# meteorologytoday/XLab-FFTBarotropic

Measured on AMD Instinct MI355X. Metric: RK4 steps/sec, 4096x4096 periodic grid, higher is better.
Workload: dtype f32; 1 GPU; 4096x4096 kuo2004 initial field, nu=6.5, L=600 km, dt=0.75 s, 4 RK stages/step, fused HIP path; parallelism=single

## Files before the change

xlab-fftbarotropic_amd/csrc/fb_col_full.h:

```cpp
#pragma once
#include "fb_kernels.h"

#define CF_THREADS 1024
#define CF_X1_CF 16384
#define CF_X2_STR 68
#define CF_X2_CF (16 * 16 * CF_X2_STR)
#define CF_GX_CF 2048
#define CF_LDS_CF (CF_X2_CF + 512 + CF_GX_CF)
#define CF_LDS_BYTES (CF_LDS_CF * 8)

struct FullArgs {
    const cf *Tin;
    const cf *Zbase;
    cf *Zcur, *Acc, *Zout;
    cf *W4;
    long fstride;
    int P;
    int ntiles;
    int ntiles_run;
    int nsub;
    int stage;
    float nu, dt;
    SpecCoef coef;
    const cf *tw256;
    const cf *tw4096;
    long sub_rows;
    float wscale;
};

FB_DEV void cf_xchg_waves(cf *lds, cf *v, int w, int lane)
{
#pragma unroll
    for (int r = 0; r < 16; ++r) lds_wr(&lds[(r * 16 + w) * 64 + lane], v[r]);
    lds_barrier();
#pragma unroll
    for (int r = 0; r < 16; ++r) v[r] = lds_rd(&lds[(w * 16 + r) * 64 + lane]);
    lds_barrier();
}

template <bool SYNC>
FB_DEV void cf_xchg_lanes(cf *lds, cf *v, int w, int l, int c)
{
    cf *reg = lds + w * (16 * CF_X2_STR);
#pragma unroll
    for (int r = 0; r < 16; ++r) lds_wr(&reg[r * CF_X2_STR + l * 4 + c], v[r]);
    __builtin_amdgcn_wave_barrier();
#pragma unroll
    for (int r = 0; r < 16; ++r) v[r] = lds_rd(&reg[l * CF_X2_STR + r * 4 + c]);
    if (SYNC) lds_barrier();
    else { asm volatile("s_waitcnt lgkmcnt(0)" ::: "memory"); __builtin_amdgcn_wave_barrier(); }
}

#define CF_FENCE() __builtin_amdgcn_sched_barrier(0)
FB_DEV cf cf_mul(cf a, cf b) { return cmul_split(a, b); }
FB_DEV cf cf_mulc(cf a, cf b) { return cmulc_split(a, b); }

template <int DIR> FB_DEV void cf_bfly16(cf *v)
{
    fft4<DIR>(v[0], v[4], v[8], v[12]);  CF_FENCE();
    fft4<DIR>(v[1], v[5], v[9], v[13]);  CF_FENCE();
    fft4<DIR>(v[2], v[6], v[10], v[14]); CF_FENCE();
    fft4<DIR>(v[3], v[7], v[11], v[15]); CF_FENCE();
    v[5]  = mul_w16<1, DIR, true>(v[5]);  v[6]  = mul_w16<2, DIR, true>(v[6]);  v[7]  = mul_w16<3, DIR, true>(v[7]);
    v[9]  = mul_w16<2, DIR, true>(v[9]);  v[10] = mul_w16<4, DIR, true>(v[10]); v[11] = mul_w16<6, DIR, true>(v[11]);
    v[13] = mul_w16<3, DIR, true>(v[13]); v[14] = mul_w16<6, DIR, true>(v[14]); v[15] = mul_w16<9, DIR, true>(v[15]);
    CF_FENCE();
    fft4<DIR>(v[0], v[1], v[2], v[3]);     CF_FENCE();
    fft4<DIR>(v[4], v[5], v[6], v[7]);     CF_FENCE();
    fft4<DIR>(v[8], v[9], v[10], v[11]);   CF_FENCE();
    fft4<DIR>(v[12], v[13], v[14], v[15]); CF_FENCE();
    cf t;
    t = v[1];  v[1]  = v[4];  v[4]  = t;
    t = v[2];  v[2]  = v[8];  v[8]  = t;
    t = v[3];  v[3]  = v[12]; v[12] = t;
    t = v[6];  v[6]  = v[9];  v[9]  = t;
    t = v[7];  v[7]  = v[13]; v[13] = t;
    t = v[11]; v[11] = v[14]; v[14] = t;
}

template <int DIR>
FB_DEV void cf_fft4096(cf *lds, const cf *tabA, const cf *tabB, cf (*v)[16], int w, int l, int c, int lane)
{
    if (DIR < 0) {
#pragma unroll
        for (int col = 0; col < 2; ++col) {
            cf_bfly16<-1>(v[col]);
#pragma unroll
            for (int k1 = 1; k1 < 16; ++k1) { v[col][k1] = cf_mul(v[col][k1], tabB[w * k1]); if ((k1 & 3) == 3) CF_FENCE(); }
            cf_xchg_waves(lds, v[col], w, lane);
            CF_FENCE();
        }
        const cf a = tabA[l * w];
#pragma unroll
        for (int col = 0; col < 2; ++col) {
            cf_bfly16<-1>(v[col]);
            v[col][0] = cf_mul(v[col][0], a);
#pragma unroll
            for (int k2 = 1; k2 < 16; ++k2) { v[col][k2] = cf_mul(v[col][k2], cf_mul(a, tabB[l * k2])); if ((k2 & 3) == 3) CF_FENCE(); }
            cf_xchg_lanes<false>(lds, v[col], w, l, c);
            CF_FENCE();
        }
#pragma unroll
        for (int col = 0; col < 2; ++col) { cf_bfly16<-1>(v[col]); CF_FENCE(); }
    } else {
#pragma unroll
        for (int col = 0; col < 2; ++col) {
            cf_bfly16<+1>(v[col]);
#pragma unroll
            for (int lr = 1; lr < 16; ++lr) { v[col][lr] = cf_mulc(v[col][lr], cf_mul(tabA[lr * w], tabB[lr * l])); if ((lr & 3) == 3) CF_FENCE(); }
            if (col == 0) cf_xchg_lanes<false>(lds, v[col], w, l, c);
            else cf_xchg_lanes<true>(lds, v[col], w, l, c);
            CF_FENCE();
        }
#pragma unroll
        for (int col = 0; col < 2; ++col) {
            cf_bfly16<+1>(v[col]);
#pragma unroll
            for (int wr = 1; wr < 16; ++wr) { v[col][wr] = cf_mulc(v[col][wr], tabB[wr * w]); if ((wr & 3) == 3) CF_FENCE(); }
            cf_xchg_waves(lds, v[col], w, lane);
            CF_FENCE();
        }
#pragma unroll
        for (int col = 0; col < 2; ++col) { cf_bfly16<+1>(v[col]); CF_FENCE(); }
    }
}

FB_DEV float4 cf_ld4(const void *ubase, unsigned voff) { return *reinterpret_cast<const float4 *>(static_cast<const char *>(ubase) + voff); }
FB_DEV void cf_st4(void *ubase, unsigned voff, float4 x) { *reinterpret_cast<float4 *>(static_cast<char *>(ubase) + voff) = x; }
FB_DEV void cf_st4_w4(void *ubase, unsigned voff, float4 x) { st4<true>(static_cast<char *>(ubase) + voff, x); }

template <int STAGE, int NSUB>
__global__ void __launch_bounds__(CF_THREADS) k_col_full(FullArgs a)
{
    extern __shared__ __attribute__((aligned(16))) unsigned char smem_raw[];
    cf *lds = reinterpret_cast<cf *>(smem_raw);
    cf *tabB = lds + CF_X2_CF, *tabA = tabB + 256;
    float *gxt = reinterpret_cast<float *>(tabA + 256);
    const int tid = threadIdx.x, lane = tid & 63, l = lane >> 2, c = lane & 3;
    const int w = __builtin_amdgcn_readfirstlane(tid >> 6);

    constexpr int nsub = NSUB;
    const int ntg = gridDim.x / nsub;
    const int k1 = NSUB == 1 ? 0 : blockIdx.x / ntg, bt = blockIdx.x - k1 * ntg;
    int tile = bt;
    if ((ntg & 7) == 0) tile = (bt & 7) * (ntg >> 3) + (bt >> 3);
    if (tile >= a.ntiles_run) return;

    const int ky0 = tile * 8 + 2 * c;
    const unsigned voff_m = (unsigned)((l * a.P + 2 * c) * (int)sizeof(cf));
    const size_t ubase_m = ((size_t)(k1 * a.sub_rows + 16 * w) * a.P + (size_t)tile * 8) * sizeof(cf);
    const size_t rstep = (size_t)256 * a.P * sizeof(cf);
    const unsigned voff_s = (unsigned)(lane * (int)sizeof(float4));
    const size_t ubase_s = ((((size_t)k1 * (a.ntiles + 1) + tile) * 16) * CF_THREADS + (size_t)w * 64) * sizeof(float4);
    const size_t sstep = (size_t)CF_THREADS * sizeof(float4);

    constexpr bool PRIME = STAGE == 4;
    cf v[2][16];
    {
        const char *src = reinterpret_cast<const char *>(a.Tin) + ubase_m;
        float4 tin[16];
        if (!PRIME) {
#pragma unroll
            for (int i = 0; i < 16; ++i) tin[i] = ld4<true>(src + i * rstep + voff_m);
        }
        float g4[4];
#pragma unroll
        for (int i = 0; i < 4; ++i) g4[i] = a.coef.gx[nsub * (tid + i * CF_THREADS) + k1];
        if (tid < 256) { tabB[tid] = a.tw256[tid]; tabA[tid] = a.tw4096[tid]; }
#pragma unroll
        for (int i = 0; i < 4; ++i) {
            const int ik = tid + i * CF_THREADS;
            gxt[((ik >> 4) & 15) + 16 * (ik & 15) + (ik & ~255)] = g4[i];
        }
        if (!PRIME) {
#pragma unroll
            for (int i = 0; i < 16; ++i) { v[0][i] = cf_make(tin[i].x, tin[i].y); v[1][i] = cf_make(tin[i].z, tin[i].w); }
        }
    }
    __syncthreads();
    if (!PRIME) cf_fft4096<-1>(lds, tabA, tabB, v, w, l, c, lane);

    const char *Z0 = reinterpret_cast<const char *>(a.Zbase) + ubase_s;
    char *ZC = reinterpret_cast<char *>(a.Zcur) + ubase_s, *AC = reinterpret_cast<char *>(a.Acc) + ubase_s,
         *ZO = reinterpret_cast<char *>(a.Zout) + ubase_s;
    const float gya = a.coef.gy[ky0], gyb = a.coef.gy[ky0 + 1];
    auto ky2_of = [](float g) { asm volatile("" : "+v"(g)); return (double)g * (double)g; };
    constexpr bool PRIME_ = STAGE == 4;
    const bool pada = PRIME_ && ky0 >= a.coef.hy, padb = PRIME_ && ky0 + 1 >= a.coef.hy;
    constexpr int stage = STAGE;
    const float nu = a.nu, dt = a.dt, hdt = (stage == 2) ? a.dt : a.dt / 2.0f;
    constexpr int DEPTH = STAGE == 0 ? 2 : 1;
#ifndef CF_REMAKE_ZC
#define CF_REMAKE_ZC 1
#endif
    constexpr bool REMAKE_ZC = CF_REMAKE_ZC && STAGE == 1;
    float4 q0[DEPTH], q1[DEPTH], q2[DEPTH];
    auto load_k3 = [&](int k3) {
        const int sl = k3 % DEPTH;
        q0[sl] = ld4<false>(Z0 + k3 * sstep + voff_s);
        if (stage != 0) q2[sl] = ld4<true>(AC + k3 * sstep + voff_s);
        if (stage != 0 && !REMAKE_ZC) q1[sl] = ld4<false>(ZC + k3 * sstep + voff_s);
    };
    if (!PRIME) {
#pragma unroll
        for (int k3 = 0; k3 < DEPTH; ++k3) load_k3(k3);
    }
#pragma unroll
    for (int k3 = 0; k3 < (PRIME ? 0 : 16); ++k3) {
        const int sl = k3 % DEPTH;
        const int ik2 = w + 256 * k3 + 16 * l, ikx = nsub * ik2 + k1;
        const float gx = gxt[l + 16 * w + 256 * k3];
        const double kx2 = (double)gx * (double)gx;
        const float lapa = (float)(-(kx2 + ky2_of(gya))), lapb = (float)(-(kx2 + ky2_of(gyb)));
        const float mska = coef_mask(a.coef, ikx, ky0), mskb = coef_mask(a.coef, ikx, ky0 + 1);
        const float4 z0 = q0[sl];
        float4 zc = z0;
        if (REMAKE_ZC) {
            const float4 ac = q2[sl];
            zc = make_float4(__builtin_fmaf(ac.x, hdt, z0.x), __builtin_fmaf(ac.y, hdt, z0.y), __builtin_fmaf(ac.z, hdt, z0.z), __builtin_fmaf(ac.w, hdt, z0.w));
        } else if (stage != 0) zc = q1[sl];
        float4 k;
        k.x = (v[0][k3].x + (zc.x * lapa) * nu) * mska; k.y = (v[0][k3].y + (zc.y * lapa) * nu) * mska;
        k.z = (v[1][k3].x + (zc.z * lapb) * nu) * mskb; k.w = (v[1][k3].y + (zc.w * lapb) * nu) * mskb;
        float4 acc, zn;
        if (stage == 0) {
            acc = k;
            zn = make_float4(__builtin_fmaf(k.x, hdt, z0.x), __builtin_fmaf(k.y, hdt, z0.y), __builtin_fmaf(k.z, hdt, z0.z), __builtin_fmaf(k.w, hdt, z0.w));
        } else if (stage < 3) {
            const float4 ac = q2[sl];
            acc = make_float4(ac.x + 2.0f * k.x, ac.y + 2.0f * k.y, ac.z + 2.0f * k.z, ac.w + 2.0f * k.w);
            zn = make_float4(z0.x + k.x * hdt, z0.y + k.y * hdt, z0.z + k.z * hdt, z0.w + k.w * hdt);
        } else {
            const float4 ac = q2[sl];
            acc = ac;
            zn = make_float4(z0.x + (ac.x + k.x) * dt / 6.0f, z0.y + (ac.y + k.y) * dt / 6.0f,
                             z0.z + (ac.z + k.z) * dt / 6.0f, z0.w + (ac.w + k.w) * dt / 6.0f);
        }
        v[0][k3] = cf_make(zn.x, zn.y); v[1][k3] = cf_make(zn.z, zn.w);
        if (k3 + DEPTH < 16) load_k3(k3 + DEPTH);
        if (stage < 3) { st4<true>(AC + k3 * sstep + voff_s, acc); cf_st4(ZC + k3 * sstep, voff_s, zn); }
        else cf_st4(ZO + k3 * sstep, voff_s, zn);
        CF_FENCE();
    }

    const char *ZN = PRIME ? Z0 : (stage < 3 ? ZC : ZO);
#pragma unroll 1
    for (int f = 0; f < 4; ++f) {
        if (f > 0 || PRIME) {
            const unsigned vs = (unsigned)launder((int)voff_s);
#pragma unroll
            for (int k3 = 0; k3 < 16; ++k3) {
                const float4 z = cf_ld4(ZN + k3 * sstep, vs);
                v[0][k3] = cf_make(z.x, z.y); v[1][k3] = cf_make(z.z, z.w);
            }
        }
        const bool psi = f >= 2, use_gx = (f == 0 || f == 3);
        const int lkx = launder(l);
#pragma unroll
        for (int k3 = 0; k3 < 16; ++k3) {
            cf za = v[0][k3], zb = v[1][k3];
            const float gx = gxt[16 * w + 256 * k3 + lkx];
            if (psi) {
                const double kx2 = (double)gx * (double)gx;
                const float lia = (nsub * (w + 256 * k3 + 16 * l) + k1 == 0 && ky0 == 0) ? 1.0f : (float)(-(kx2 + ky2_of(gya)));
                const float lib = (float)(-(kx2 + ky2_of(gyb)));
                za = pada ? cf_make(0.f, 0.f) : cf_make(za.x / lia, za.y / lia);
                zb = padb ? cf_make(0.f, 0.f) : cf_make(zb.x / lib, zb.y / lib);
            }
            const float ka = (use_gx ? gx : gya) * a.wscale, kb = (use_gx ? gx : gyb) * a.wscale;
            v[0][k3] = cf_make(-za.y * ka, za.x * ka);
            v[1][k3] = cf_make(-zb.y * kb, zb.x * kb);
            CF_FENCE();
        }
        cf_fft4096<+1>(lds, tabA, tabB, v, w, l, c, lane);
        char *dst = reinterpret_cast<char *>(a.W4) + (size_t)f * a.fstride * sizeof(cf) + ubase_m;
        const unsigned vm = (unsigned)launder((int)voff_m);
#pragma unroll
        for (int i = 0; i < 16; ++i)
            cf_st4_w4(dst + i * rstep, vm, make_float4(v[0][i].x, v[0][i].y, v[1][i].x, v[1][i].y));
    }
}

template <bool TO_FULL>
__global__ void __launch_bounds__(256) k_full_relayout(const cf *__restrict__ in, cf *__restrict__ out, int P, int N1, int N2, int ntiles, int nsub, int hy)
{
    const size_t total = (size_t)nsub * (ntiles + 1) * 16 * CF_THREADS * 2;
    for (size_t idx = (size_t)blockIdx.x * blockDim.x + threadIdx.x; idx < total; idx += (size_t)gridDim.x * blockDim.x) {
        const int col = (int)(idx & 1);
        const int tid = (int)((idx >> 1) & (CF_THREADS - 1));
        const int k3 = (int)((idx >> 11) & 15);
        const int st = (int)(idx >> 15);
        const int k1 = st / (ntiles + 1), tile = st - k1 * (ntiles + 1);
        const int w = tid >> 6, l = (tid >> 2) & 15, c = tid & 3;
        const int kx = nsub * (w + 16 * l + 256 * k3) + k1, ky = tile * 8 + 2 * c + col;
        const int cc = kx % N1, d = kx / N1;
        const size_t p3 = (size_t)(N2 * cc + d) * P + ky;
        if (ky >= hy) { if (TO_FULL) out[idx] = cf_make(0.f, 0.f); continue; }
        if (TO_FULL) out[idx] = in[p3]; else out[p3] = in[idx];
    }
}
```

xlab-fftbarotropic_amd/csrc/fb_kernels.h:

```cpp
#pragma once
#include "fb_fft_core.h"

struct SpecCoef {
    const float  *gx;
    const double *kx2;
    const float  *gy;
    const double *ky2;
    double gws;
    int nx, hy;
    int gws_i;
};

FB_DEV float coef_lap(const SpecCoef &c, int i, int j) { return (float)(-(c.kx2[i] + c.ky2[j])); }
FB_DEV float coef_mask(const SpecCoef &c, int i, int j)
{
    const int ii = i < c.nx - i ? i : c.nx - i;
    const int r2 = ii * ii + j * j;
    return (r2 >= c.gws_i || j >= c.hy) ? 0.0f : 1.0f;
}

enum { OP_GRADX = 0, OP_GRADY = 1, OP_LAP = 2, OP_INVLAP = 3, OP_DEALIAS = 4 };

template <int OP>
__global__ void __launch_bounds__(256) k_spec_op(SpecCoef c, const cf *__restrict__ in, cf *__restrict__ out, int hy, size_t total)
{
#pragma clang fp contract(off)
    for (size_t idx = (size_t)blockIdx.x * blockDim.x + threadIdx.x; idx < total; idx += (size_t)gridDim.x * blockDim.x) {
        const int i = (int)(idx / hy), j = (int)(idx - (size_t)i * hy);
        cf a = in[idx], r;
        if (OP == OP_GRADX) { float k = c.gx[i]; r = cf_make(-a.y * k, a.x * k); }
        else if (OP == OP_GRADY) { float k = c.gy[j]; r = cf_make(-a.y * k, a.x * k); }
        else if (OP == OP_LAP) { float k = coef_lap(c, i, j); r = cf_make(a.x * k, a.y * k); }
        else if (OP == OP_INVLAP) { float k = (i == 0 && j == 0) ? 1.0f : coef_lap(c, i, j);
                                    r = cf_make(a.x / k, a.y / k); }
        else { float k = coef_mask(c, i, j); r = cf_make(a.x * k, a.y * k); }
        out[idx] = r;
    }
}

__global__ void __launch_bounds__(256) k_scale_real(float *d, float s, int divide, size_t n)
{
#pragma clang fp contract(off)
    for (size_t i = (size_t)blockIdx.x * blockDim.x + threadIdx.x; i < n; i += (size_t)gridDim.x * blockDim.x)
        d[i] = divide ? d[i] / s : d[i] * s;
}

__global__ void __launch_bounds__(256) k_jacobian(const float *__restrict__ u, const float *__restrict__ v,
                                                  const float *__restrict__ dx, const float *__restrict__ dy,
                                                  const float *__restrict__ src, float *__restrict__ out, size_t n)
{
#pragma clang fp contract(off)
    for (size_t i = (size_t)blockIdx.x * blockDim.x + threadIdx.x; i < n; i += (size_t)gridDim.x * blockDim.x) {
        float s = src ? src[i] : 0.0f;
        out[i] = -u[i] * dx[i] - v[i] * dy[i] + s;
    }
}

__global__ void __launch_bounds__(256) k_spec_axpy(const float *__restrict__ base, const float *__restrict__ x, float a,
                                                   float *__restrict__ out, size_t n)
{
#pragma clang fp contract(off)
    for (size_t i = (size_t)blockIdx.x * blockDim.x + threadIdx.x; i < n; i += (size_t)gridDim.x * blockDim.x)
        out[i] = base[i] + x[i] * a;
}

__global__ void __launch_bounds__(256) k_rk4_combine(const float *__restrict__ base, const float *__restrict__ k1,
                                                     const float *__restrict__ k2, const float *__restrict__ k3,
                                                     const float *__restrict__ k4, float dt, float *__restrict__ out, size_t n)
{
#pragma clang fp contract(off)
    for (size_t i = (size_t)blockIdx.x * blockDim.x + threadIdx.x; i < n; i += (size_t)gridDim.x * blockDim.x)
        out[i] = base[i] + (k1[i] + 2.0f * k2[i] + 2.0f * k3[i] + k4[i]) * dt / 6.0f;
}

template <bool TO_PRIVATE>
__global__ void __launch_bounds__(256) k_spec_relayout(const cf *__restrict__ in, cf *__restrict__ out, int nx, int hy, int P, int N1, int N2)
{
    const size_t total = (size_t)nx * P;
    for (size_t idx = (size_t)blockIdx.x * blockDim.x + threadIdx.x; idx < total; idx += (size_t)gridDim.x * blockDim.x) {
        const int row = (int)(idx / P), col = (int)(idx - (size_t)row * P);
        const int c = row / N2, d = row - c * N2, kx = c + N1 * d;
        if (TO_PRIVATE) out[idx] = col < hy ? in[(size_t)kx * hy + col] : cf_make(0.f, 0.f);
        else if (col < hy) out[(size_t)kx * hy + col] = in[idx];
    }
}

template <int MODE>
__global__ void __launch_bounds__(256) k_psi_private(SpecCoef c, cf *__restrict__ z, int P, int N1, int N2, int ky0)
{
#pragma clang fp contract(off)
    const size_t total = (size_t)c.nx * P;
    for (size_t idx = (size_t)blockIdx.x * blockDim.x + threadIdx.x; idx < total; idx += (size_t)gridDim.x * blockDim.x) {
        const int row = (int)(idx / P), col = (int)(idx - (size_t)row * P);
        const int cc = row / N2, d = row - cc * N2, i = cc + N1 * d, j = ky0 + col;
        cf a = z[idx];
        if (j >= c.hy) { z[idx] = cf_make(0.f, 0.f); continue; }
        const float li = (i == 0 && j == 0) ? 1.0f : coef_lap(c, i, j);
        a = cf_make(a.x / li, a.y / li);
        if (MODE == 1) { const float k = c.gy[j]; a = cf_make(-a.y * k, a.x * k); }
        if (MODE == 2) { const float k = c.gx[i]; a = cf_make(-a.y * k, a.x * k); }
        z[idx] = a;
    }
}

__global__ void __launch_bounds__(256) k_ow_spec(SpecCoef c, const cf *zin, cf *z, long fstride, int P, int N1, int N2, int ky0)
{
#pragma clang fp contract(off)
    const size_t total = (size_t)c.nx * P;
    for (size_t idx = (size_t)blockIdx.x * blockDim.x + threadIdx.x; idx < total; idx += (size_t)gridDim.x * blockDim.x) {
        const int row = (int)(idx / P), col = (int)(idx - (size_t)row * P);
        const int cc = row / N2, d = row - cc * N2, i = cc + N1 * d, j = ky0 + col;
        cf a = zin[idx], xx = cf_make(0.f, 0.f), yy = xx, xy = xx;
        if (j < c.hy) {
            const float li = (i == 0 && j == 0) ? 1.0f : coef_lap(c, i, j);
            a = cf_make(a.x / li, a.y / li);
            const float kx = c.gx[i], ky = c.gy[j];
            const cf ax = cf_make(-a.y * kx, a.x * kx), ay = cf_make(-a.y * ky, a.x * ky);
            xx = cf_make(-ax.y * kx, ax.x * kx);
            yy = cf_make(-ay.y * ky, ay.x * ky);
            xy = cf_make(-ay.y * kx, ay.x * kx);
        }
        z[idx] = xx; z[idx + fstride] = yy; z[idx + 2 * fstride] = xy;
    }
}

__global__ void __launch_bounds__(256) k_pres_spec(SpecCoef c, const cf *zin, cf *z, long fstride, int P, int N1, int N2, int ky0)
{
#pragma clang fp contract(off)
    const size_t total = (size_t)c.nx * P;
    for (size_t idx = (size_t)blockIdx.x * blockDim.x + threadIdx.x; idx < total; idx += (size_t)gridDim.x * blockDim.x) {
        const int row = (int)(idx / P), col = (int)(idx - (size_t)row * P);
        const int cc = row / N2, d = row - cc * N2, i = cc + N1 * d, j = ky0 + col;
        cf a = zin[idx], xx = cf_make(0.f, 0.f), yy = xx, xy = xx;
        if (j < c.hy) {
            const float li = (i == 0 && j == 0) ? 1.0f : coef_lap(c, i, j);
            a = cf_make(a.x / li, a.y / li);
            const float kx = c.gx[i], ky = c.gy[j], mk = coef_mask(c, i, j);
            const cf ax = cf_make(-a.y * kx, a.x * kx), ay = cf_make(-a.y * ky, a.x * ky);
            xx = cf_make(-ax.y * kx, ax.x * kx);
            yy = cf_make(-ay.y * ky, ay.x * ky);
            xy = cf_make(-ay.y * kx, ay.x * kx);
            xx = cf_make(xx.x * mk, xx.y * mk);
            yy = cf_make(yy.x * mk, yy.y * mk);
            xy = cf_make(xy.x * mk, xy.y * mk);
        }
        z[idx] = xx; z[idx + fstride] = yy; z[idx + 2 * fstride] = xy;
    }
}

__global__ void __launch_bounds__(256) k_pres_solve(SpecCoef c, const cf *__restrict__ zin, cf *__restrict__ l, float rho, float f, int P, int N1, int N2,
                                                    int ky0)
{
#pragma clang fp contract(off)
    const size_t total = (size_t)c.nx * P;
    for (size_t idx = (size_t)blockIdx.x * blockDim.x + threadIdx.x; idx < total; idx += (size_t)gridDim.x * blockDim.x) {
        const int row = (int)(idx / P), col = (int)(idx - (size_t)row * P);
        const int cc = row / N2, d = row - cc * N2, i = cc + N1 * d, j = ky0 + col;
        if (j >= c.hy) { l[idx] = cf_make(0.f, 0.f); continue; }
        const float lap = coef_lap(c, i, j), li = (i == 0 && j == 0) ? 1.0f : lap;
        const cf v = zin[idx], L = l[idx];
        const cf psi = cf_make(v.x / li, v.y / li);
        const cf t = cf_make(psi.x * lap, psi.y * lap);
        const float ax = t.x * f, ay = t.y * f, bx = L.x + L.x, by = L.y + L.y;
        const float qx = rho * (bx + ax), qy = rho * (by + ay);
        l[idx] = cf_make(qx / li, qy / li);
    }
}

__global__ void k_pres_ref(const float *__restrict__ p, long at, float *__restrict__ dst, int world)
{
    const int i = blockIdx.x * blockDim.x + threadIdx.x;
    if (i < world) dst[i] = at >= 0 ? p[at] : 0.0f;
}
template <bool V4>
__global__ void __launch_bounds__(256) k_pres_sub(float *__restrict__ p, size_t n, const float *__restrict__ ref)
{
    const float r = *ref;
    const size_t stride = (size_t)gridDim.x * blockDim.x;
    if (V4) {
        float4 *p4 = reinterpret_cast<float4 *>(p);
        for (size_t i = (size_t)blockIdx.x * blockDim.x + threadIdx.x; i < n / 4; i += stride) {
            float4 v = p4[i];
            v.x -= r; v.y -= r; v.z -= r; v.w -= r;
            p4[i] = v;
        }
    } else {
        for (size_t i = (size_t)blockIdx.x * blockDim.x + threadIdx.x; i < n; i += stride) p[i] -= r;
    }
}

template <bool TO_TM>
__global__ void __launch_bounds__(256) k_state_relayout(const cf *__restrict__ in, cf *__restrict__ out, int nx, int P, int N2)
{
    const int R1 = N2 >> 3, NLB = N2 >> 2, ntc = P >> 4;
    const size_t total = (size_t)nx * P;
    for (size_t idx = (size_t)blockIdx.x * blockDim.x + threadIdx.x; idx < total; idx += (size_t)gridDim.x * blockDim.x) {
        const int row = (int)(idx / P), col = (int)(idx - (size_t)row * P);
        const int cb = row / N2, d = row - cb * N2, ct = col >> 4, c = col & 15;
        const int q = d / R1, rem = d - q * R1, h = rem & 3, sidx = rem >> 2, e = 8 * sidx + q;
        const size_t tile = (size_t)cb * ntc + ct;
        const size_t tm = ((tile * (NLB / 2) + (e >> 1)) * 64 + (16 * h + c)) * 2 + (e & 1);
        if (TO_TM) out[tm] = in[idx]; else out[idx] = in[tm];
    }
}

enum { ROW_FUSED = 0, ROW_INV = 1, ROW_FWD = 2, ROW_OW = 3, ROW_KEFF = 4, ROW_PRES = 5 };

FB_DEV float pres_curv_point(float pxx, float pyy, float pxy)
{
#pragma clang fp contract(off)
    const float a = pxx * pyy, b = pxy * pxy;
    return a - b;
}

FB_DEV void ow_point(float pxx, float pyy, float pxy, float *w_out, float *tau_out, size_t i)
{
#pragma clang fp contract(off)
    const float w = 4.0f * (pxy * pxy - pxx * pyy);
    if (w_out) w_out[i] = w;
    if (tau_out) tau_out[i] = w > 0.0f ? 2.0f / sqrtf(w) : __builtin_inff();
}

FB_DEV void keff_grad2_point(float zx, float zy, float *g_out, size_t i)
{
#pragma clang fp contract(off)
    g_out[i] = zx * zx + zy * zy;
}

struct RowView {
    const cf *a, *b, *f;
    long fstrA, fstrB, fstrF;
    long sstrA, sstrB, sstrF;
    int ka, ka0, kb, kf;
    int katot;
    unsigned magA, magF;
};
struct RowArgs {
    RowView M;
    RowView T;
    int t_frozen;
    const float *src;
    const int *src_nz;
    const float *rin;
    float *rout;
    int x0, nx;
    float scale;
    int prescaled;
    const cf *tw_bwd, *tw_fwd;
    long sub_rows;
    const cf *tw_x;
};

FB_DEV float *row_rout2(const RowArgs &a) { return const_cast<float *>(a.rin); }

__global__ void __launch_bounds__(256) k_src_row_flags(const float *__restrict__ src, int *__restrict__ flags, int ny)
{
    const float4 *row = reinterpret_cast<const float4 *>(src + (size_t)blockIdx.x * ny);
    int any = 0;
    for (int i = threadIdx.x; i < ny / 4; i += 256) { const float4 v = row[i]; any |= (v.x != 0.f) | (v.y != 0.f) | (v.z != 0.f) | (v.w != 0.f); }
    any = __syncthreads_or(any);
    if (threadIdx.x == 0) flags[blockIdx.x] = any ? 1 : 0;
}

template <int N> struct RowCfg {
    static constexpr int T = N / 16;
    static constexpr int G = T >= 256 ? 1 : 256 / T;
    static constexpr int THREADS = T * G;
    static constexpr bool HALFX = false;
    static constexpr int LSTR = HALFX ? (N / 2 + N / 32) : (N + N / 16);
    static constexpr bool DMA = N >= 1024 && N <= 8192;
    static constexpr int GSTR = LSTR + (DMA ? N : 0);
    static constexpr bool RES = RowRes<N>::value;
    static constexpr bool SHARE = RES && RowPlanSymmetric<N>::value;
    static constexpr int TWL_B = RowTwSrc<N, false, RES>::LDS_CF, TWL_F = SHARE ? 0 : RowTwSrc<N, true, RES>::LDS_CF;
    static constexpr bool PAIR2 = N <= 1024 && G >= 2;
    static constexpr int VALB = PAIR2 ? G * 8 * T : 0;
    static constexpr size_t LDS_BYTES = ((size_t)G * GSTR + TWL_B + TWL_F + VALB) * sizeof(cf);
    static constexpr int MIN_WAVES = HALFX ? 3 : (THREADS == 256 ? 2 : (THREADS == 512 ? 2 : 4));
};

template <bool SLAB>
FB_DEV const cf *row_ptr(const RowView &v, int field, int row, int k)
{
    if (!SLAB) return v.a + (size_t)field * v.fstrA + (size_t)row * v.ka + k;
    if (k < v.katot) {
        const int s = (int)__umulhi((unsigned)k, v.magA), w = k - s * v.ka;
        if (v.kb == 0) return v.a + (size_t)field * v.fstrA + (size_t)s * v.sstrA + (size_t)row * v.ka + w;
        const bool inb = w >= v.ka0;
        const cf *base = inb ? v.b : v.a;
        const long fstr = inb ? v.fstrB : v.fstrA, sstr = inb ? v.sstrB : v.sstrA;
        const int kc = inb ? v.kb : v.ka0, wc = inb ? w - v.ka0 : w;
        return base + (size_t)field * fstr + (size_t)s * sstr + (size_t)row * kc + wc;
    }
    const int kk = k - v.katot, s = (int)__umulhi((unsigned)kk, v.magF);
    return v.f + (size_t)field * v.fstrF + (size_t)s * v.sstrF + (size_t)row * v.kf + (kk - s * v.kf);
}
template <bool SLAB> FB_DEV bool row_keep(const RowView &v, int t_frozen, int k) { return !SLAB || t_frozen || k < v.katot; }

template <int N, bool SLAB, int TAG = 0>
FB_DEV void row_load_pair(cf *reg, int t, const RowView &v, int fA, int fB, int rowA, int rowB)
{
    constexpr int T = N / 16, R0 = RowTw<N, false>::radix(0);
#pragma unroll
    for (int e = 0; e < 16; ++e) {
        const int i = ord_i<R0>(e);
        if (i < 8) {
            const int k = t + i * T;
            const cf a = *row_ptr<SLAB>(v, fA, rowA, k), b = *row_ptr<SLAB>(v, fB, rowB, k);
            reg[e] = (i == 0 && t == 0) ? cf_make(a.x, b.x) : cf_make(a.x - b.y, a.y + b.x);
        } else {
            const int k = (16 - i) * T - t;
            const cf a = *row_ptr<SLAB>(v, fA, rowA, k), b = *row_ptr<SLAB>(v, fB, rowB, k);
            reg[e] = (i == 8 && t == 0) ? cf_make(a.x, b.x) : cf_make(a.x + b.y, b.x - a.y);
        }
    }
}

template <int N, bool SLAB>
FB_DEV void row_store_pair(cf *lds, int t, const cf *reg, bool valid, const RowView &v, int t_frozen, int rowA, int rowB)
{
    constexpr int T = N / 16, RL = RowTw<N, true>::radix(RowPlan<N>::S - 1);
    constexpr int HOFF = RowCfg<N>::HALFX ? N / 2 : 0;
// ... 619 lines not shown
```

xlab-fftbarotropic_amd/csrc/fftbaro.hip:

```cpp
#include <hip/hip_runtime.h>
#include <algorithm>
#include <cmath>
#include <cstdio>
#include <cstdlib>
#include <cstring>
#include <mutex>
#include <set>
#include <string>
#include <type_traits>
#include <utility>
#include <vector>

#include "../../include/fftbaro.h"
#include "fb_kernels.h"
#include "fb_keff.h"
#include "fb_azim.h"
#include "fb_census.h"
#include "fb_spectra.h"
#include "fb_tracer.h"
#include "fb_particles.h"
#include "fb_tangent.h"
#include "fb_adjoint.h"
#include "fb_col_full.h"
#include "fb_row3.h"
// ... 767 lines not shown
        if (verbose) fprintf(stderr, "fftbaro: pitch probe P=%d %.4f ms\n", P0 + 16 * k, tbest[k]);
        if (tbest[k] < best * 0.99f) { best = tbest[k]; bestP = P0 + 16 * k; }
    }
    if (verbose) fprintf(stderr, "fftbaro: pitch %d -> %d\n", P0, bestP);
    c->P = c->KA = c->katot = c->grp[0].ncols = bestP;
    finish_groups(c);
    hipEventDestroy(e0); hipEventDestroy(e1);
    hipFree(buf);
    hipGetLastError();
    return FB_OK;
}

static int ensure_scratch(fb_ctx *c)
{
    if (!c->d_scratch) {
        hipError_t e = hipMalloc((void **)&c->d_scratch, priv_elems(c) * sizeof(cf));
        if (e != hipSuccess) return fail(FB_ENOMEM, "scratch allocation failed");
    }
    return FB_OK;
}

static unsigned magic_div(int d) { return d > 0 ? (unsigned)((1ull << 32) / (unsigned)d) + 1u : 0u; }
static RowView view_single(const fb_ctx *c, const cf *base, long fstride)
{
    RowView v; memset(&v, 0, sizeof(v));
    v.a = v.b = v.f = base; v.fstrA = v.fstrB = v.fstrF = fstride; v.ka = v.ka0 = c->P; v.kb = 0; v.kf = 16; v.katot = 0x7fffffff;
    return v;
}
static RowView view_slab(const fb_ctx *c, const cf *const *bufs, int nfields)
{
    RowView v; memset(&v, 0, sizeof(v));
    v.a = bufs[0]; v.b = c->nact > 1 ? bufs[1] : bufs[0]; v.f = c->KF > 0 ? bufs[c->nact] : bufs[0];
    v.ka = c->KA; v.ka0 = c->grp[0].ncols; v.kb = c->nact > 1 ? c->grp[1].ncols : 0; v.kf = c->KF > 0 ? c->KF : 16;
    v.katot = c->katot;
    v.fstrA = (long)c->XL * v.ka0; v.fstrB = (long)c->XL * v.kb; v.fstrF = (long)c->XL * v.kf;
    v.sstrA = (long)nfields * v.fstrA; v.sstrB = (long)nfields * v.fstrB; v.sstrF = (long)nfields * v.fstrF;
    v.magA = magic_div(v.ka); v.magF = magic_div(v.kf);
    return v;
}
static RowArgs row_args_base(const fb_ctx *c)
{
    RowArgs a; memset(&a, 0, sizeof(a));
    a.x0 = 0; a.nx = c->XL; a.tw_bwd = c->d_tw_row_bwd; a.tw_fwd = c->d_tw_row_fwd; a.t_frozen = 1;
    return a;
}

static int r2c_private(fb_ctx *c, const float *d_real, cf *dst)
{
    RowArgs a = row_args_base(c); a.rin = d_real; a.T = view_single(c, dst, 0);
    int rc;
    if ((rc = launch_row<ROW_FWD>(c, a))) return rc;
    if ((rc = launch_col_strided<-1>(c, c->grp[0], dst, 1, 0))) return rc;
    return launch_col_block<-1>(c, c->grp[0], dst, 1, 0);
}

static int c2r_private(fb_ctx *c, cf *work, float *d_real, float scale)
{
    int rc;
    if ((rc = launch_col_block<+1>(c, c->grp[0], work, 1, 0))) return rc;
    if ((rc = launch_col_strided<+1>(c, c->grp[0], work, 1, 0))) return rc;
    RowArgs a = row_args_base(c); a.M = view_single(c, work, 0); a.rout = d_real; a.scale = scale;
    return launch_row<ROW_INV>(c, a);
}

static bool state_tm(const fb_ctx *c) { return c->N2 >= 32; }
static int state_convert(fb_ctx *c, const ColGroup &G, const cf *in, cf *out, bool to_tm)
{
    if (G.ncols == 0) return FB_OK;
    if (!state_tm(c)) { HIPCHK(hipMemcpyAsync(out, in, grp_elems(c, G) * sizeof(cf), hipMemcpyDeviceToDevice, c->stream)); return FB_OK; }
    const size_t total = grp_elems(c, G);
    return launch_n(c, to_tm ? k_state_relayout<true> : k_state_relayout<false>, total, in, out, c->nx, G.ncols, c->N2);
}

static int relayout(fb_ctx *c, const cf *in, cf *out, bool to_private)
{
    const size_t total = priv_elems(c);
    return launch_n(c, to_private ? k_spec_relayout<true> : k_spec_relayout<false>, total, in, out, c->nx, c->hy, c->P, c->N1, c->N2);
}

extern "C" int fb_r2c(fb_ctx *c, const float *d_in, float *d_out)
{
    if (!c || !d_in || !d_out) return fail(FB_EINVAL, "fb_r2c: NULL");
    NEED_SINGLE(c);
    int rc;
    if ((rc = ensure_scratch(c))) return rc;
    HIPCHK(hipMemsetAsync(c->d_scratch, 0, priv_elems(c) * sizeof(cf), c->stream));
    if ((rc = r2c_private(c, d_in, c->d_scratch))) return rc;
    return relayout(c, c->d_scratch, (cf *)d_out, false);
}

extern "C" int fb_c2r(fb_ctx *c, const float *d_in, float *d_out, int normalize)
{
    if (!c || !d_in || !d_out) return fail(FB_EINVAL, "fb_c2r: NULL");
    NEED_SINGLE(c);
    int rc;
    if ((rc = ensure_scratch(c))) return rc;
    if ((rc = relayout(c, (const cf *)d_in, c->d_scratch, true))) return rc;
    const float scale = normalize ? 1.0f / (float)((size_t)c->nx * c->ny) : 1.0f;
    return c2r_private(c, c->d_scratch, d_out, scale);
}

struct GroupBufs { cf *ZA, *ZB, *ACC, *w4_send, *w4_recv, *t_send, *t_recv; };

struct Beside { cf *c0[3], *c1[3], *acc[3]; };

struct fb_model {
    fb_ctx *c;
    float nu, dt;
    GroupBufs gb[3];
    bool phase_flow;
    XPass xpass;
    bool prescale;
    bool use_graph, warmed;
    hipGraphExec_t graph_exec;
    const float *graph_src; hipStream_t graph_stream;
    float *src;
    int *src_nz;
    cf *rec_work[3], *rec_send[3];
    float *keff_fields;
    void *keff_red; size_t keff_red_cap;
    float *azim_fields;
    void *azim_red; size_t azim_red_cap;
    int *cs_label, *cs_ids;
    int2 *cs_part;
    float *pres_ref;
    unsigned char rec_work_nf[3], rec_send_nf[3];
    void *spec_red;
    int primed;
    Beside tr;
    float kappa;
    bool tracer;
    double *pt; int pt_n;
    float *pt_uv;
    double *pd;
    long long steps, pd_steps0;
    Beside tg[FB_TANGENTS_MAX];
    int tg_n;
    cf *tg_j[3];
    double *tg_red;
    cf *ad_tape; int ad_depth, ad_fill;
    Beside ad;
    float *ad_real;
    bool adjoint;
};

#include "fb_transport.h"
struct fb_slab {
    fb_ctx *c;
    fb_model *m;
    fb_transport tp;
    bool connected, owns_streams;
    hipStream_t comp, comm;
    hipEvent_t ev_f[4], ev_r[8], ev_w4, ev_t, ev_tg[2], ev_rows_done, ev_fwd_done, ev_misc[2];
    int nfg, nch;
    int ncg;
    int step_ops;
};
#include "fb_entry.h"

static int model_create_impl(fb_model **out, fb_ctx *c, float nu, float dt, bool phase_flow)
{
    if (!out || !c) return fail(FB_EINVAL, "fb_model_create: NULL");
    *out = nullptr;
    fb_model *m = new fb_model();
    memset(m, 0, sizeof(*m));
    m->c = c; m->nu = nu; m->dt = dt; m->phase_flow = phase_flow;
    m->xpass = phase_flow ? XP_COLS : choose_xpass(c);
    m->prescale = m->xpass != XP_COLS && c->world == 1 && c->row == RK_ROWQ && !c->no_prescale;
    int rc = FB_OK;
    auto alloc0 = [&](cf **p, size_t elems) {
        if (rc || elems == 0) return;
        if (hipMalloc((void **)p, elems * sizeof(cf)) != hipSuccess) { rc = fail(FB_ENOMEM, "model allocation failed"); return; }
        if (hipMemsetAsync(*p, 0, elems * sizeof(cf), c->stream) != hipSuccess) rc = fail(FB_EHIP, "hipMemsetAsync failed");
    };
    for (int g = 0; g < c->ngroups; ++g) {
        const size_t n = grp_elems(c, c->grp[g]);
        GroupBufs &B = m->gb[g];
        alloc0(&B.ZA, n);
        if (g < c->nact) { alloc0(&B.ZB, n); alloc0(&B.ACC, n); }
        alloc0(&B.w4_send, 4 * n); alloc0(&B.t_send, n);
        if (c->world > 1) { alloc0(&B.w4_recv, 4 * n); alloc0(&B.t_recv, n); }
        else { B.w4_recv = B.w4_send; B.t_recv = B.t_send; }
    }
    if (rc) { fb_model_destroy(m); return rc; }
    *out = m;
    return FB_OK;
}

extern "C" int fb_model_create(fb_model **out, fb_ctx *c, float nu, float dt)
{
    if (c && c->world != 1) return fail(FB_EINVAL, "fb_model_create on a slab context: use fb_slab_create");
    return model_create_impl(out, c, nu, dt, false);
}

static int beside_stage(fb_model *m, fb_slab *s, int stage);
static void beside_step_done(fb_model *m);
static void beside_free_all(fb_model *m);

static void model_drop_graph(fb_model *m)
{
    if (m->graph_exec) { hipGraphExecDestroy(m->graph_exec); m->graph_exec = nullptr; }
}

static void state_replaced(fb_model *m)
{
    m->warmed = false;
    m->primed = 0;
    m->ad_fill = 0;
}

extern "C" int fb_model_destroy(fb_model *m)
{
    if (!m) return FB_OK;
    for (GroupBufs &B : m->gb) {
        if (B.w4_recv && B.w4_recv != B.w4_send) hipFree(B.w4_recv);
        if (B.t_recv && B.t_recv != B.t_send) hipFree(B.t_recv);
        cf *arr[] = {B.ZA, B.ZB, B.ACC, B.w4_send, B.t_send};
        for (cf *p : arr) if (p) hipFree(p);
    }
    model_drop_graph(m);
    if (m->src) hipFree(m->src);
    if (m->src_nz) hipFree(m->src_nz);
    for (auto p : m->rec_work) if (p) hipFree(p);
    for (auto p : m->rec_send) if (p) hipFree(p);
    if (m->keff_fields) hipFree(m->keff_fields);
    if (m->keff_red) hipFree(m->keff_red);
    if (m->azim_fields) hipFree(m->azim_fields);
    if (m->azim_red) hipFree(m->azim_red);
    if (m->cs_label) hipFree(m->cs_label);
    if (m->cs_ids) hipFree(m->cs_ids);
    if (m->cs_part) hipFree(m->cs_part);
    if (m->pres_ref) hipFree(m->pres_ref);
    if (m->spec_red) hipFree(m->spec_red);
    beside_free_all(m);
    delete m;
    return FB_OK;
}

extern "C" int fb_model_info(fb_model *m, size_t *hbm, size_t *alg)
{
    if (int rc = enter(on_model("fb_model_info", m))) return rc;
    const fb_ctx *c = m->c;
    if (hbm) {
        size_t n = m->src ? (size_t)c->XL * c->ny * 4 : 0;
        for (int g = 0; g < c->ngroups; ++g) n += (c->world > 1 ? (g < c->nact ? 13 : 11) : 8) * grp_elems(c, c->grp[g]) * sizeof(cf);
        for (int g = 0; g < c->ngroups && m->tracer; ++g) n += (g < c->nact ? 3 : 1) * grp_elems(c, c->grp[g]) * sizeof(cf);
        if (m->pt_n) n += 6 * (size_t)m->pt_n * sizeof(double) + 2 * (size_t)c->nx * c->ny * sizeof(float);
        if (m->pd) n += 12 * (size_t)m->pt_n * sizeof(double);
        for (int g = 0; g < c->ngroups && m->tg_n; ++g)
            n += ((size_t)m->tg_n * (g < c->nact ? 3 : 1) + (g < c->nact ? 1 : 0)) * grp_elems(c, c->grp[g]) * sizeof(cf);
        if (m->cs_label) n += 2 * (size_t)c->nx * c->ny * sizeof(int);
        if (m->cs_part) n += (size_t)c->nx * c->ny / CENSUS_TILE * sizeof(int2);
        *hbm = n;
    }
    if (alg) *alg = (size_t)320 * c->nx * c->ny;
    return FB_OK;
}

static int set_source(const Call &k, const float *d_src)
{
    if (int rc = enter(k)) return rc;
    fb_model *m = k.m;
    fb_ctx *c = m->c;
    const size_t n = (size_t)c->XL * c->ny * sizeof(float);
    if (!d_src) { if (m->src) { HIPCHK(hipStreamSynchronize(c->stream)); hipFree(m->src); m->src = nullptr; } return FB_OK; }
    if (!m->src_nz && hipMalloc((void **)&m->src_nz, (size_t)c->XL * sizeof(int)) != hipSuccess) { m->src_nz = nullptr; return fail(FB_ENOMEM, "source allocation failed"); }
    if (!m->src && hipMalloc((void **)&m->src, n) != hipSuccess) { m->src = nullptr; return fail(FB_ENOMEM, "source allocation failed"); }
    if (int rc = launch(c, k_src_row_flags, dim3(c->XL), dim3(256), 0, d_src, m->src_nz, c->ny)) return rc;
    const size_t half = (size_t)c->XL * c->ny / 2;
    switch (c->row) {
    case RK_ROWQ: return launch_n(c, k_rowq_permute_src, half, d_src, m->src, c->XL);
    case RK_ROWH_8192: return launch_n(c, k_rowh_permute_src<1>, half, d_src, m->src, c->XL);
    case RK_ROWH_16384: return launch_n(c, k_rowh_permute_src<2>, half, d_src, m->src, c->XL);
    default: HIPCHK(hipMemcpyAsync(m->src, d_src, n, hipMemcpyDeviceToDevice, c->stream)); return FB_OK;
    }
}
extern "C" int fb_model_set_source(fb_model *m, const float *d_src) { return set_source(on_model("fb_model_set_source", m), d_src); }
extern "C" int fb_slab_set_source_local(fb_slab *s, const float *d_rows) { return set_source(on_slab("fb_slab_set_source_local", s), d_rows); }

static MidArgs mid_args(fb_model *m, int g, int stage)
{
    fb_ctx *c = m->c;
    const ColGroup &G = c->grp[g];
    const GroupBufs &B = m->gb[g];
    MidArgs a;
    a.Tin = B.t_recv; a.Zbase = B.ZA; a.Zcur = B.ZB; a.Acc = B.ACC; a.Zout = B.ZA; a.W4 = B.w4_send;
    a.ct0 = 0; a.nct = stage < 0 ? G.ncols / 16 : G.nct_active;
    a.fstride = w4_fstride(c, G); a.rm = rowmap_w4(c, G); a.P = G.ncols; a.N1 = c->N1; a.N2 = c->N2; a.ky0 = G.ky0; a.stage = stage;
    a.nu = m->nu; a.dt = m->dt; a.coef = make_coef(c); a.tw_n = c->d_tw_n2; a.tw_big = c->d_tw_big;
    return a;
}

static int launch_col_full(fb_model *m, int stage)
{
    fb_ctx *c = m->c;
    const GroupBufs &B = m->gb[0];
    FullArgs a;
    a.Tin = B.t_recv; a.Zbase = B.ZA; a.Zcur = B.ZB; a.Acc = B.ACC; a.Zout = B.ZA; a.W4 = B.w4_send;
    a.fstride = (long)priv_elems(c); a.P = c->P; a.ntiles = (c->ny / 2) / 8; a.stage = stage; a.nu = m->nu; a.dt = m->dt;
    a.nsub = m->xpass; a.sub_rows = 4096;
    a.wscale = m->prescale ? 1.0f / (float)((size_t)c->nx * c->ny) : 1.0f;
    a.ntiles_run = c->grp[0].nct_active * 2 < a.ntiles ? c->grp[0].nct_active * 2 : a.ntiles;
    if (c->full_noskip) a.ntiles_run = a.ntiles;
    if (stage == 4) a.ntiles_run = a.ntiles + 1;
    a.coef = make_coef(c); a.tw256 = c->d_tw_256; a.tw4096 = m->xpass == XP_FULL1 ? c->d_tw_big : c->d_tw_4096;
    return launch_full(c, a);
}

static int full_import_state(fb_model *m, cf *spec3)
{
    fb_ctx *c = m->c;
    const int ntiles = (c->ny / 2) / 8;
    int rc;
    if ((rc = launch(c, k_full_relayout<true>, dim3(c->max_wg), dim3(256), 0, (const cf *)spec3, m->gb[0].ZA, c->P, c->N1, c->N2, ntiles, (int)m->xpass, c->hy)) ||
        (rc = launch_col_full(m, 4)))
        return rc;
    m->primed = 2;
    return FB_OK;
}

static int full_export_state(fb_model *m, cf *dst)
{
    fb_ctx *c = m->c;
    HIPCHK(hipMemsetAsync(dst, 0, priv_elems(c) * sizeof(cf), c->stream));
    const int ntiles = (c->ny / 2) / 8;
    return launch(c, k_full_relayout<false>, dim3(c->max_wg), dim3(256), 0, (const cf *)m->gb[0].ZA, dst, c->P, c->N1, c->N2, ntiles, (int)m->xpass, c->hy);
}

static int export_state(fb_model *m, int g, cf *dst)
{
    return m->xpass != XP_COLS ? full_export_state(m, dst) : state_convert(m->c, m->c->grp[g], m->gb[g].ZA, dst, false);
}

static int model_prime(fb_model *m)
{
    fb_ctx *c = m->c;
    int rc;
    for (int g = 0; g < c->ngroups; ++g) {
        const ColGroup &G = c->grp[g];
        if ((rc = launch_col_mid(c, mid_args(m, g, -1)))) return rc;
        if ((rc = launch_col_strided<+1>(c, G, m->gb[g].w4_send, 4, w4_fstride(c, G), rowmap_w4(c, G), G.nct_active, G.ncols / 16 - G.nct_active))) return rc;
    }
    m->primed = 1;
    return FB_OK;
}
static int model_col_bwd_active(fb_model *m, int f0 = 0, int f1 = 4, int g = 0)
{
    fb_ctx *c = m->c;
    const ColGroup &G = c->grp[g];
    return launch_col_strided<+1>(c, G, m->gb[g].w4_send + (size_t)f0 * w4_fstride(c, G), f1 - f0, w4_fstride(c, G), rowmap_w4(c, G), 0, G.nct_active);
}
static int launch_fused_row(fb_model *m, int x0, int nrows)
{
    fb_ctx *c = m->c;
    RowArgs a = row_args_base(c);
    if (c->world == 1) { a.M = view_single(c, m->gb[0].w4_recv, (long)priv_elems(c)); a.T = view_single(c, m->gb[0].t_send, 0); }
    else {
        const cf *w4[3] = {m->gb[0].w4_recv, m->gb[1].w4_recv, m->gb[2].w4_recv}, *ts[3] = {m->gb[0].t_send, m->gb[1].t_send, m->gb[2].t_send};
        a.M = view_slab(c, w4, 4); a.T = view_slab(c, ts, 1); a.t_frozen = 0;
    }
    a.src = m->src; a.src_nz = m->src_nz; a.scale = 1.0f / (float)((size_t)c->nx * c->ny); a.x0 = x0; a.nx = nrows; a.prescaled = m->prescale ? 1 : 0;
    return launch_row<ROW_FUSED>(c, a, m->xpass == XP_FULL2 ? RK_ROWH2 : c->row);
}
static int model_col_fwd(fb_model *m, int stage, int g = 0)
{
    fb_ctx *c = m->c;
    int rc;
    if ((rc = launch_col_strided<-1>(c, c->grp[g], m->gb[g].t_recv, 1, 0, rowmap_natural(), 0, c->grp[g].nct_active))) return rc;
    m->primed = 1;
    return launch_col_mid(c, mid_args(m, g, stage));
}

struct StepProf {
    std::vector<hipEvent_t> ev0[4], ev1[4];
    hipStream_t stream;
    int begin(int cls) { hipEvent_t a, b; if (hipEventCreate(&a) != hipSuccess || hipEventCreate(&b) != hipSuccess) return 1;
                         ev0[cls].push_back(a); ev1[cls].push_back(b); return hipEventRecord(a, stream) != hipSuccess; }
    int end(int cls) { return hipEventRecord(ev1[cls].back(), stream) != hipSuccess; }
};
#define PROF_BEGIN(cls) do { if (prof && prof->begin(cls)) return fail(FB_EHIP, "event record failed"); } while (0)
#define PROF_END(cls) do { if (prof && prof->end(cls)) return fail(FB_EHIP, "event record failed"); } while (0)

static int step_refusals(const Call &k, int nsteps)
{
    if (nsteps < 0) return refuse(k, "bad argument: nsteps < 0");
    if (int rc = enter(k, NEED_TRANSPORT)) return rc;
    const fb_model *m = k.m;
    if (m->ad_depth && nsteps > m->ad_depth - m->ad_fill)
        return refuse(k, "the adjoint's tape has room for " + std::to_string(m->ad_depth - m->ad_fill) + " more steps (fb_model_adjoint_record)");
    return FB_OK;
}

static int model_step_impl(fb_model *m, int nsteps, StepProf *prof)
{
    fb_ctx *c = m->c;
    int rc;
    if (nsteps == 0) return FB_OK;
    if (m->xpass != XP_COLS && !m->primed) return fail(FB_EINVAL, "fb_model_step: set the state first");
    if (!m->primed && (rc = model_prime(m))) return rc;
    if (m->primed == 1 && m->xpass == XP_COLS) { if ((rc = model_col_bwd_active(m))) return rc; m->primed = 2; }
    const ColGroup &G = c->grp[0];
    GroupBufs &B = m->gb[0];
    for (int s = 0; s < nsteps; ++s) {
        for (int k = 0; k < 4; ++k) {
            if ((rc = beside_stage(m, nullptr, k))) return rc;
            PROF_BEGIN(1);
            if ((rc = launch_fused_row(m, 0, c->XL))) return rc;
            PROF_END(1);
            if (m->xpass != XP_COLS) {
                PROF_BEGIN(3);
                if ((rc = launch_col_full(m, k))) return rc;
                PROF_END(3);
                continue;
            }
            PROF_BEGIN(2);
            if ((rc = launch_col_strided<-1>(c, G, B.t_recv, 1, 0, rowmap_natural(), 0, G.nct_active))) return rc;
            PROF_END(2);
            PROF_BEGIN(3);
            if ((rc = launch_col_mid(c, mid_args(m, 0, k)))) return rc;
            PROF_END(3);
            PROF_BEGIN(0);
            if ((rc = launch_col_strided<+1>(c, G, B.w4_send, 4, (long)priv_elems(c), rowmap_natural(), 0, G.nct_active))) return rc;
            PROF_END(0);
        }
        beside_step_done(m);
    }
    return FB_OK;
}

extern "C" int fb_model_use_graph(fb_model *m, int enable)
{
    if (int rc = enter(on_model("fb_model_use_graph", m))) return rc;
    m->use_graph = enable != 0;
    if (!m->use_graph) model_drop_graph(m);
    return FB_OK;
}

static int model_steps(fb_model *m, int nsteps)
{
    fb_ctx *c = m->c;
    if (!m->use_graph || c->world != 1 || c->stream == nullptr || nsteps < 2 || m->ad_depth) { if (nsteps > 0) m->warmed = true; return model_step_impl(m, nsteps, nullptr); }
    int rc;
    if (!m->warmed) { if ((rc = model_step_impl(m, 1, nullptr))) return rc; m->warmed = true; --nsteps; }
    if (m->graph_exec && (m->graph_src != m->src || m->graph_stream != c->stream)) model_drop_graph(m);
    if (!m->graph_exec) {
        hipGraph_t g = nullptr;
        HIPCHK(hipStreamBeginCapture(c->stream, hipStreamCaptureModeThreadLocal));
        rc = model_step_impl(m, 1, nullptr);
        hipError_t e = hipStreamEndCapture(c->stream, &g);
        if (rc) { if (g) hipGraphDestroy(g); return rc; }
        HIPCHK(e);
        e = hipGraphInstantiate(&m->graph_exec, g, nullptr, nullptr, 0);
        hipGraphDestroy(g);
        HIPCHK(e);
        m->graph_src = m->src; m->graph_stream = c->stream;
    }
    for (int s = 0; s < nsteps; ++s) HIPCHK(hipGraphLaunch(m->graph_exec, c->stream));
    return FB_OK;
}

extern "C" int fb_model_profile_steps(fb_model *m, int nsteps, float *ms_sum, int *launches)
{
    const Call k = on_model("fb_model_profile_steps", m);
    if (!ms_sum || !launches) return refuse(k, "NULL output");
    int rc;
    if ((rc = step_refusals(k, nsteps))) return rc;
    StepProf prof; prof.stream = m->c->stream;
    rc = model_step_impl(m, nsteps, &prof);
    if (!rc) m->steps += nsteps;
    HIPCHK(hipStreamSynchronize(m->c->stream));
    for (int cls = 0; cls < 4; ++cls) {
        ms_sum[cls] = 0.f; launches[cls] = (int)prof.ev0[cls].size();
        for (size_t i = 0; i < prof.ev0[cls].size(); ++i) {
            float ms = 0.f;
            if (i < prof.ev1[cls].size() && hipEventElapsedTime(&ms, prof.ev0[cls][i], prof.ev1[cls][i]) == hipSuccess) ms_sum[cls] += ms;
            hipEventDestroy(prof.ev0[cls][i]);
            if (i < prof.ev1[cls].size()) hipEventDestroy(prof.ev1[cls][i]);
        }
    }
    return rc;
}

extern "C" int fb_model_get_spectrum(fb_model *m, float *d_spec)
{
    const Call k = on_model("fb_model_get_spectrum", m);
    if (!d_spec) return refuse(k, "NULL output");
    int rc;
    if ((rc = enter(k, NEED_TRANSPORT))) return rc;
    if ((rc = ensure_scratch(m->c))) return rc;
    if ((rc = export_state(m, 0, m->c->d_scratch))) return rc;
    return relayout(m->c, m->c->d_scratch, (cf *)d_spec, false);
}

extern "C" int fb_model_set_spectrum(fb_model *m, const float *d_spec)
{
    const Call k = on_model("fb_model_set_spectrum", m);
    if (!d_spec) return refuse(k, "NULL input");
    int rc;
    if ((rc = enter(k, NEED_TRANSPORT))) return rc;
    state_replaced(m);
    rc = relayout(m->c, (const cf *)d_spec, m->gb[0].ZB, true);
    if (rc) return rc;
    if (m->xpass != XP_COLS) return full_import_state(m, m->gb[0].ZB);
    return state_convert(m->c, m->c->grp[0], m->gb[0].ZB, m->gb[0].ZA, true);
}

#include "fb_slab_driver.h"
#include "fb_record.h"
#include "fb_beside.h"
```

Measured before the change: 1213 steps/s.

## Skip Acc/Zcur traffic for fully dealiased spectral slabs in fused column kernel

For each k3 slab the kernel now checks whether every mode the wave owns lies outside the dealiasing mask. For such frozen slabs it turns the Acc/Zcur loads and stores into no-ops by passing a zero-size buffer resource, keeps zn equal to z0, and later reads the base field instead of the never-written output. It also changes the tile-to-block mapping for NSUB==2 so blocks are interleaved differently. This is meant to cut memory bandwidth on masked high-wavenumber regions, at the cost of extra mask checks and reliance on raw buffer intrinsics with out-of-range suppression.

```diff
diff --git a/xlab-fftbarotropic_amd/csrc/fb_col_full.h b/xlab-fftbarotropic_amd/csrc/fb_col_full.h
--- a/xlab-fftbarotropic_amd/csrc/fb_col_full.h
+++ b/xlab-fftbarotropic_amd/csrc/fb_col_full.h
@@ -26,6 +26,7 @@
     const cf *tw4096;
     long sub_rows;
     float wscale;
+    int noskip;
 };
 
 FB_DEV void cf_xchg_waves(cf *lds, cf *v, int w, int lane)
@@ -129,6 +130,27 @@
 FB_DEV void cf_st4(void *ubase, unsigned voff, float4 x) { *reinterpret_cast<float4 *>(static_cast<char *>(ubase) + voff) = x; }
 FB_DEV void cf_st4_w4(void *ubase, unsigned voff, float4 x) { st4<true>(static_cast<char *>(ubase) + voff, x); }
 
+typedef float cf_f4v __attribute__((ext_vector_type(4)));
+typedef int cf_i4v __attribute__((ext_vector_type(4)));
+__device__ cf_f4v cf_raw_buffer_load(cf_i4v rsrc, int voffset, int soffset, int aux) __asm("llvm.amdgcn.raw.buffer.load.v4f32");
+__device__ void cf_raw_buffer_store(cf_f4v data, cf_i4v rsrc, int voffset, int soffset, int aux) __asm("llvm.amdgcn.raw.buffer.store.v4f32");
+FB_DEV cf_i4v cf_wave_rsrc(const void *ubase, bool live)
+{
+    const unsigned long long b = reinterpret_cast<unsigned long long>(ubase);
+    const cf_i4v r = {(int)(unsigned)b, (int)(unsigned)(b >> 32), live ? 64 * (int)sizeof(float4) : 0, 0x00020000 };
+    return r;
+}
+template <bool NT> FB_DEV float4 cf_ldw(const void *ubase, bool live, unsigned voff)
+{
+    const cf_f4v x = cf_raw_buffer_load(cf_wave_rsrc(ubase, live), (int)voff, 0, NT ? 2 : 0);
+    return make_float4(x.x, x.y, x.z, x.w);
+}
+template <bool NT> FB_DEV void cf_stw(void *ubase, bool live, unsigned voff, float4 x)
+{
+    const cf_f4v d = {x.x, x.y, x.z, x.w};
+    cf_raw_buffer_store(d, cf_wave_rsrc(ubase, live), (int)voff, 0, NT ? 2 : 0);
+}
+
 template <int STAGE, int NSUB>
 __global__ void __launch_bounds__(CF_THREADS) k_col_full(FullArgs a)
 {
@@ -143,7 +165,8 @@
     const int ntg = gridDim.x / nsub;
     const int k1 = NSUB == 1 ? 0 : blockIdx.x / ntg, bt = blockIdx.x - k1 * ntg;
     int tile = bt;
-    if ((ntg & 7) == 0) tile = (bt & 7) * (ntg >> 3) + (bt >> 3);
+    if (NSUB == 2 && (ntg & 15) == 0) tile = 2 * (8 * (bt >> 4) + (bt & 7)) + ((bt >> 3) & 1);
+    else if ((ntg & 7) == 0) tile = (bt & 7) * (ntg >> 3) + (bt >> 3);
     if (tile >= a.ntiles_run) return;
 
     const int ky0 = tile * 8 + 2 * c;
@@ -156,12 +179,19 @@
 
     constexpr bool PRIME = STAGE == 4;
     cf v[2][16];
+    unsigned frozen = 0;
     {
         const char *src = reinterpret_cast<const char *>(a.Tin) + ubase_m;
         float4 tin[16];
         if (!PRIME) {
 #pragma unroll
             for (int i = 0; i < 16; ++i) tin[i] = ld4<true>(src + i * rstep + voff_m);
+#pragma unroll
+            for (int k3 = 0; k3 < 16; ++k3) {
+                const int kxlo = nsub * (w + 256 * k3) + k1, kxhi = nsub * (w + 256 * k3 + 16 * 15) + k1;
+                frozen |= (unsigned)(coef_masked(a.coef, kxlo, tile * 8) & coef_masked(a.coef, kxhi, tile * 8)) << k3;
+            }
+            if (a.noskip) frozen = 0;
         }
         float g4[4];
 #pragma unroll
@@ -195,11 +225,13 @@
 #endif
     constexpr bool REMAKE_ZC = CF_REMAKE_ZC && STAGE == 1;
     float4 q0[DEPTH], q1[DEPTH], q2[DEPTH];
+    auto frozen_k3 = [&](int k3) { return (frozen >> k3 & 1u) != 0; };
     auto load_k3 = [&](int k3) {
         const int sl = k3 % DEPTH;
         q0[sl] = ld4<false>(Z0 + k3 * sstep + voff_s);
-        if (stage != 0) q2[sl] = ld4<true>(AC + k3 * sstep + voff_s);
-        if (stage != 0 && !REMAKE_ZC) q1[sl] = ld4<false>(ZC + k3 * sstep + voff_s);
+        const bool live = !frozen_k3(k3);
+        if (stage != 0) q2[sl] = cf_ldw<true>(AC + k3 * sstep, live, voff_s);
+        if (stage != 0 && !REMAKE_ZC) q1[sl] = cf_ldw<false>(ZC + k3 * sstep, live, voff_s);
     };
     if (!PRIME) {
 #pragma unroll
@@ -236,10 +268,12 @@
             zn = make_float4(z0.x + (ac.x + k.x) * dt / 6.0f, z0.y + (ac.y + k.y) * dt / 6.0f,
                              z0.z + (ac.z + k.z) * dt / 6.0f, z0.w + (ac.w + k.w) * dt / 6.0f);
         }
+        const bool live = !frozen_k3(k3);
+        if (!live) zn = z0;
         v[0][k3] = cf_make(zn.x, zn.y); v[1][k3] = cf_make(zn.z, zn.w);
         if (k3 + DEPTH < 16) load_k3(k3 + DEPTH);
-        if (stage < 3) { st4<true>(AC + k3 * sstep + voff_s, acc); cf_st4(ZC + k3 * sstep, voff_s, zn); }
-        else cf_st4(ZO + k3 * sstep, voff_s, zn);
+        if (stage < 3) { cf_stw<true>(AC + k3 * sstep, live, voff_s, acc); cf_stw<false>(ZC + k3 * sstep, live, voff_s, zn); }
+        else cf_stw<false>(ZO + k3 * sstep, live, voff_s, zn);
         CF_FENCE();
     }
 
@@ -250,7 +284,8 @@
             const unsigned vs = (unsigned)launder((int)voff_s);
 #pragma unroll
             for (int k3 = 0; k3 < 16; ++k3) {
-                const float4 z = cf_ld4(ZN + k3 * sstep, vs);
+                const char *zsrc = (!PRIME && stage < 3 && frozen_k3(k3)) ? Z0 : ZN;
+                const float4 z = cf_ld4(zsrc + k3 * sstep, vs);
                 v[0][k3] = cf_make(z.x, z.y); v[1][k3] = cf_make(z.z, z.w);
             }
         }
diff --git a/xlab-fftbarotropic_amd/csrc/fb_kernels.h b/xlab-fftbarotropic_amd/csrc/fb_kernels.h
--- a/xlab-fftbarotropic_amd/csrc/fb_kernels.h
+++ b/xlab-fftbarotropic_amd/csrc/fb_kernels.h
@@ -12,12 +12,13 @@
 };
 
 FB_DEV float coef_lap(const SpecCoef &c, int i, int j) { return (float)(-(c.kx2[i] + c.ky2[j])); }
-FB_DEV float coef_mask(const SpecCoef &c, int i, int j)
+FB_DEV bool coef_masked(const SpecCoef &c, int i, int j)
 {
     const int ii = i < c.nx - i ? i : c.nx - i;
     const int r2 = ii * ii + j * j;
-    return (r2 >= c.gws_i || j >= c.hy) ? 0.0f : 1.0f;
-}
+    return r2 >= c.gws_i || j >= c.hy;
+}
+FB_DEV float coef_mask(const SpecCoef &c, int i, int j) { return coef_masked(c, i, j) ? 0.0f : 1.0f; }
 
 enum { OP_GRADX = 0, OP_GRADY = 1, OP_LAP = 2, OP_INVLAP = 3, OP_DEALIAS = 4 };
 
diff --git a/xlab-fftbarotropic_amd/csrc/fftbaro.hip b/xlab-fftbarotropic_amd/csrc/fftbaro.hip
--- a/xlab-fftbarotropic_amd/csrc/fftbaro.hip
+++ b/xlab-fftbarotropic_amd/csrc/fftbaro.hip
@@ -1093,6 +1093,7 @@
     a.wscale = m->prescale ? 1.0f / (float)((size_t)c->nx * c->ny) : 1.0f;
     a.ntiles_run = c->grp[0].nct_active * 2 < a.ntiles ? c->grp[0].nct_active * 2 : a.ntiles;
     if (c->full_noskip) a.ntiles_run = a.ntiles;
+    a.noskip = c->full_noskip;
     if (stage == 4) a.ntiles_run = a.ntiles + 1;
     a.coef = make_coef(c); a.tw256 = c->d_tw_256; a.tw4096 = m->xpass == XP_FULL1 ? c->d_tw_big : c->d_tw_4096;
     return launch_full(c, a);
```

After: 1226 steps/s, median of 6. About the same (+1.0%).
